# gvanhorn38/multibox

Measured on AMD Instinct MI355X. Metric: images/sec (299x299, 5-AR priors) train, higher is better.
Workload: dtype bf16; 1 GPU; full train step: Inception-ResNet-v2 + multibox heads fwd, on-device matching+loss, bwd, RMSProp+EMA; 299x299, k=5 (P=646), BATCH_SIZE=64/GPU, MAX_NUM_BBOXES=13; global_batch=64, parallelism=dp1, hip_graph=True

## Files before the change

multibox_amd/csrc/bn.hip:

```cpp
#include "vec8.h"
#include <string.h>
#include <type_traits>

namespace {

__device__ __forceinline__ void block_sum2(double& s1, double& s2) {
  __shared__ double red[kT / 64][2];
  s1 = wave_sum(s1); s2 = wave_sum(s2);
  if ((threadIdx.x & 63) == 0) { red[threadIdx.x >> 6][0] = s1; red[threadIdx.x >> 6][1] = s2; }
  __syncthreads();
  s1 = red[0][0] + red[1][0] + red[2][0] + red[3][0];
  s2 = red[0][1] + red[1][1] + red[2][1] + red[3][1];
}

__device__ __forceinline__ double bn_mean_var(double s1, double s2, double inv_count, double& var) {
  const double m = s1 * inv_count;
  var = s2 * inv_count - m * m;
  if (var < 0.0) var = 0.0;
  return m;
}
__device__ __forceinline__ float bn_rstd(double var, float eps) { return (float)(1.0 / sqrt(var + (double)eps)); }
__device__ __forceinline__ void bn_publish(int c, float fm, float fr, double var, float decay, float* mean,
                                           float* rstd, float* mmean, float* mvar) {
  mean[c] = fm;
// ... 445 lines not shown
      const float2 v1 = *reinterpret_cast<const float2*>(src + (size_t)(r + 1) * C * 2);
      const float2 v2 = *reinterpret_cast<const float2*>(src + (size_t)(r + 2) * C * 2);
      const float2 v3 = *reinterpret_cast<const float2*>(src + (size_t)(r + 3) * C * 2);
      s1 += ((double)v0.x + (double)v1.x) + ((double)v2.x + (double)v3.x);
      s2 += ((double)v0.y + (double)v1.y) + ((double)v2.y + (double)v3.y);
    }
    for (; r < rows; ++r) {
      const float2 v = *reinterpret_cast<const float2*>(src + (size_t)r * C * 2);
      s1 += v.x; s2 += v.y;
    }
    const float mu = mean[ch], rs = rstd[ch];
    const double sgx = (double)rs * (s2 - (double)mu * s1);
    s_par[ch] = mu; s_par[C + ch] = rs; s_par[2 * C + ch] = thr[ch];
    s_par[3 * C + ch] = (float)(s1 * inv_M); s_par[4 * C + ch] = (float)(sgx * inv_M);
    if (blockIdx.x == 0 && dbeta) dbeta[ch] += (float)s1;
  }
  __syncthreads();
  if (!active) return;
  float mu[8], rs[8], th[8], m1[8], m2[8];
#pragma unroll
  for (int j = 0; j < 8; ++j) {
    mu[j] = s_par[c + j]; rs[j] = s_par[C + c + j]; th[j] = s_par[2 * C + c + j]; m1[j] = s_par[3 * C + c + j]; m2[j] = s_par[4 * C + c + j];
  }
  u32x4 gc = g0, yc = y0;
  for (; m < M; m += step) {
    u32x4 gn = u32x4{0u, 0u, 0u, 0u}, yn = u32x4{0u, 0u, 0u, 0u};
    if (m + step < M) { gn = ld8(dap + (m + step) * ld_da); yn = ld8(y + (m + step) * C + c); }
    float g[8], yy[8], o[8];
    unpack8(gc, g);
    unpack8(yc, yy);
#pragma unroll
    for (int j = 0; j < 8; ++j)
      o[j] = bn_bwd_value(g[j], bn_xhat(yy[j], mu[j], rs[j]), yy[j] > th[j], rs[j], m1[j], m2[j]);
    st8(dy + m * C + c, pack8(o));
    gc = gn; yc = yn;
  }
}

inline unsigned rows_launch_grid(long long M, int C) {
  static const int rows_blocks = mbx_env_int("MBX_BN_ROWS_BLOCKS", 1024);
  const int C8 = C / 8, rpi = kT / C8 > 0 ? kT / C8 : 1;
  const long long g = (M + rpi - 1) / rpi;
  return (unsigned)(g > rows_blocks ? rows_blocks : g);
}

inline void bn_fused_grid(long long M, int C, int rows, int& groups, int& chunks, int& rpc) {
  groups = (C + kBnGroup - 1) / kBnGroup;
  static const int blocks_few = mbx_env_int("MBX_BN_FUSED_BLOCKS", 1024), blocks_many = mbx_env_int("MBX_BN_FUSED_BLOCKS_MANY", 256);
  long long want = (rows > 16 ? blocks_many : blocks_few) / groups;
  if (want < 1) want = 1;
  long long maxc = (M + 255) / 256;
  if (want > maxc) want = maxc;
  rpc = (int)((M + want - 1) / want);
  chunks = (int)((M + rpc - 1) / rpc);
}

#ifndef MBX_OB_SLOTS
#define MBX_OB_SLOTS 8
#endif
#ifndef MBX_OB_SLEEP
#define MBX_OB_SLEEP 8
#endif
constexpr int kObT = 512;
constexpr int kObSlots = MBX_OB_SLOTS;
constexpr int kObMaxNV = 20;
#ifndef MBX_OB_SUB
#define MBX_OB_SUB 16
#endif
#ifndef MBX_OB_REL
#define MBX_OB_REL 32
#endif
constexpr int kObSub = MBX_OB_SUB, kObRel = MBX_OB_REL, kObLine = 32;
constexpr int kObCtlWords = kObLine * (2 + kObSub + kObRel);

struct ObGeom { int C8, rpi, G, rpb, nv; };
inline ObGeom ob_geom(long long M, int C, int ncu) {
  ObGeom g;
  g.C8 = C / 8;
  g.rpi = g.C8 <= kObT ? kObT / g.C8 : 0;
  if (g.rpi == 0) { g.G = g.rpb = 0; g.nv = 1 << 30; return g; }
  long long G = (M + g.rpi - 1) / g.rpi;
  if (G > ncu) G = ncu;
  g.rpb = (int)((M + G - 1) / G);
  g.G = (int)((M + g.rpb - 1) / g.rpb);
  g.nv = (g.rpb + g.rpi - 1) / g.rpi;
  return g;
}

__device__ __forceinline__ unsigned ld_agent(const unsigned* p) {
  return __hip_atomic_load(p, __ATOMIC_RELAXED, __HIP_MEMORY_SCOPE_AGENT);
}
__device__ __forceinline__ float ld_agent(const float* p) {
  return __hip_atomic_load(p, __ATOMIC_RELAXED, __HIP_MEMORY_SCOPE_AGENT);
}

__device__ __forceinline__ __amdgpu_buffer_rsrc_t ob_rsrc(const void* p, unsigned bytes) {
  return __builtin_amdgcn_make_buffer_rsrc(const_cast<void*>(p), (short)0, (int)bytes, 0x00020000);
}
__device__ __forceinline__ u32x4 ob_load16(__amdgpu_buffer_rsrc_t r, unsigned byte_off) {
  return __builtin_amdgcn_raw_buffer_load_b128(r, (int)byte_off, 0, 0);
}
__device__ __forceinline__ void ob_store16(__amdgpu_buffer_rsrc_t r, unsigned byte_off, u32x4 v) {
  __builtin_amdgcn_raw_buffer_store_b128(v, r, (int)byte_off, 0, 0);
}

template <int NC, int NR>
__device__ __forceinline__ void ob_sum_cols(const float* p, int cstride, int ncols, int rstride, int nrows, float (&t)[NC]) {
#pragma unroll
  for (int k = 0; k < NC; ++k) t[k] = 0.f;
  for (int r0 = 0; r0 < nrows; r0 += NR) {
    float v[NC][NR];
#pragma unroll
    for (int k = 0; k < NC; ++k) {
      const int ko = (k < ncols ? k : 0) * cstride;
#pragma unroll
      for (int r = 0; r < NR; ++r) v[k][r] = p[ko + (r0 + r < nrows ? r0 + r : nrows - 1) * rstride];
    }
#pragma unroll
    for (int r = 0; r < NR; ++r) {
      const bool in = r0 + r < nrows;
#pragma unroll
      for (int k = 0; k < NC; ++k) t[k] += in ? v[k][r] : 0.f;
    }
  }
}

template <int NC, int NR>
__device__ __forceinline__ void ob_reduce_wide(const float* rows, int C2, int rpi, float* acc) {
  for (int e0 = threadIdx.x; e0 < C2; e0 += NC * kObT) {
    const int ncols = (C2 - e0 + kObT - 1) / kObT;
    float t[NC];
    ob_sum_cols<NC, NR>(rows + e0, kObT, ncols, C2, rpi, t);
#pragma unroll
    for (int k = 0; k < NC; ++k)
      if (k < ncols) atomicAdd(acc + e0 + k * kObT, t[k]);
  }
}

template <int NV, bool RELU>
__global__ void __launch_bounds__(kObT)
bn_bwd_onepass_kernel(const unsigned short* __restrict__ da, int ld_da, const unsigned short* __restrict__ y,
                      long long M, int C, const float* __restrict__ mean, const float* __restrict__ rstd,
                      const float* __restrict__ beta, float* __restrict__ dbeta, unsigned short* __restrict__ dy,
                      float* __restrict__ ws, int rpi, int rpb, float inv_M, unsigned spin_limit, int fault,
                      float* __restrict__ step_poison, const ChanMap map, int map_max) {
  extern __shared__ __attribute__((aligned(16))) float sred[];
  __shared__ int s_timeout;
  const int C8 = C >> 3;
  const int vc = threadIdx.x % C8, rr = threadIdx.x / C8;
  const bool active = rr < rpi;
  const int c = vc << 3;
  const long long r0 = (long long)((fault & 2) ? xcd_logical((int)blockIdx.x, (int)gridDim.x) : (int)blockIdx.x) * rpb;
  long long nr = (r0 + rpb > M ? M : r0 + rpb) - r0;
  const int nrows = nr > 0 ? (int)nr : 0;
  const __amdgpu_buffer_rsrc_t gr = ob_rsrc(da + r0 * ld_da, nrows ? (unsigned)(((nrows - 1) * ld_da + C + map_max) * 2) : 0u);
  const int cg = c + chan_off(map, c);
  const __amdgpu_buffer_rsrc_t yr = ob_rsrc(y + r0 * C, (unsigned)(nrows * C * 2));
  const __amdgpu_buffer_rsrc_t dr = ob_rsrc(dy + r0 * C, (unsigned)(nrows * C * 2));
  constexpr unsigned kPast = 0x80000000u;
  u32x4 vg[NV], vy[NV];
#pragma unroll
  for (int i = 0; i < NV; ++i) {
    const int lr = rr + i * rpi;
    const bool ok = active && lr < nrows;
    vg[i] = ob_load16(gr, ok ? (unsigned)((lr * ld_da + cg) * 2) : kPast);
    vy[i] = ob_load16(yr, ok ? (unsigned)((lr * C + c) * 2) : kPast);
  }
  float s1[8], s2[8], mu[8], rs[8], be[8];
  {
    const int cs = active ? c : 0;
    const float4 a0 = *reinterpret_cast<const float4*>(mean + cs), a1 = *reinterpret_cast<const float4*>(mean + cs + 4);
    const float4 b0 = *reinterpret_cast<const float4*>(rstd + cs), b1 = *reinterpret_cast<const float4*>(rstd + cs + 4);
    mu[0] = a0.x; mu[1] = a0.y; mu[2] = a0.z; mu[3] = a0.w; mu[4] = a1.x; mu[5] = a1.y; mu[6] = a1.z; mu[7] = a1.w;
    rs[0] = b0.x; rs[1] = b0.y; rs[2] = b0.z; rs[3] = b0.w; rs[4] = b1.x; rs[5] = b1.y; rs[6] = b1.z; rs[7] = b1.w;
    if (RELU) {
      const float4 c0 = *reinterpret_cast<const float4*>(beta + cs), c1 = *reinterpret_cast<const float4*>(beta + cs + 4);
      be[0] = c0.x; be[1] = c0.y; be[2] = c0.z; be[3] = c0.w; be[4] = c1.x; be[5] = c1.y; be[6] = c1.z; be[7] = c1.w;
    } else {
#pragma unroll
      for (int j = 0; j < 8; ++j) be[j] = 0.f;
    }
#pragma unroll
    for (int j = 0; j < 8; ++j) { s1[j] = 0.f; s2[j] = 0.f; }
  }
#pragma unroll
  for (int i = 0; i < NV; ++i) {
    asm volatile("" : "+v"(vg[i]), "+v"(vy[i]));
    float g[8], yy[8];
    unpack8(vg[i], g);
    unpack8(vy[i], yy);
#pragma unroll
    for (int j = 0; j < 8; ++j) {
      const float xh = bn_xhat(yy[j], mu[j], rs[j]);
      const float gj = (!RELU || bn_pre_relu(xh, be[j]) > 0.f) ? g[j] : 0.f;
      s1[j] += gj;
      s2[j] += gj * xh;
    }
    asm volatile("" : "+v"(s1[0]), "+v"(s1[1]), "+v"(s1[2]), "+v"(s1[3]), "+v"(s1[4]), "+v"(s1[5]), "+v"(s1[6]), "+v"(s1[7]));
    asm volatile("" : "+v"(s2[0]), "+v"(s2[1]), "+v"(s2[2]), "+v"(s2[3]), "+v"(s2[4]), "+v"(s2[5]), "+v"(s2[6]), "+v"(s2[7]));
  }
  const int C2 = 2 * C;
  if (active) {
    float4* o1 = reinterpret_cast<float4*>(sred + (size_t)rr * C2 + c);
    float4* o2 = reinterpret_cast<float4*>(sred + (size_t)rr * C2 + C + c);
    o1[0] = make_float4(s1[0], s1[1], s1[2], s1[3]); o1[1] = make_float4(s1[4], s1[5], s1[6], s1[7]);
    o2[0] = make_float4(s2[0], s2[1], s2[2], s2[3]); o2[1] = make_float4(s2[4], s2[5], s2[6], s2[7]);
  }
  __syncthreads();
  float* acc = ws + (size_t)(blockIdx.x & (kObSlots - 1)) * 2 * C;
  unsigned* ctl = reinterpret_cast<unsigned*>(ws + (size_t)kObSlots * 2 * C);
  const int np = C2 < kObT ? kObT / C2 : 1;
  if (np > 1) {
    float* part = sred + (size_t)rpi * C2;
    const int e = threadIdx.x % C2, p = threadIdx.x / C2;
    float t[1];
    if (p < np) {
      ob_sum_cols<1, 16>(sred + p * C2 + e, 0, 1, np * C2, (rpi - p + np - 1) / np, t);
      part[p * C2 + e] = t[0];
    }
    __syncthreads();
    if (threadIdx.x < C2) {
      ob_sum_cols<1, 16>(part + threadIdx.x, 0, 1, C2, np, t);
      atomicAdd(acc + threadIdx.x, t[0]);
    }
  } else if (rpi > 8) ob_reduce_wide<1, 16>(sred, C2, rpi, acc);
  else if (rpi > 4) ob_reduce_wide<2, 8>(sred, C2, rpi, acc);
  else if (rpi > 2) ob_reduce_wide<4, 4>(sred, C2, rpi, acc);
  else if (rpi > 1) ob_reduce_wide<8, 2>(sred, C2, rpi, acc);
  else ob_reduce_wide<16, 1>(sred, C2, rpi, acc);
  asm volatile("s_waitcnt vmcnt(0) lgkmcnt(0)" ::: "memory");
  __syncthreads();
  if (threadIdx.x == 0) {
    const unsigned G = gridDim.x, b = blockIdx.x;
    const unsigned sub = b % kObSub, n_sub = (G - sub + kObSub - 1) / kObSub, n_top = G < kObSub ? G : kObSub;
    s_timeout = 0;
    bool last = ((fault & 1) && b == 0) ? false : atomicAdd(ctl + kObLine * (1 + sub), 1u) == n_sub - 1;
    if (last) last = atomicAdd(ctl + kObLine * (1 + kObSub), 1u) == n_top - 1;
    if (last) {
      for (int r = 0; r < kObRel; ++r)
        __hip_atomic_store(ctl + kObLine * (2 + kObSub + r), 1u, __ATOMIC_RELAXED, __HIP_MEMORY_SCOPE_AGENT);
    } else {
      const unsigned* rel = ctl + kObLine * (2 + kObSub + b % kObRel);
      unsigned spins = 0;
      while (ld_agent(rel) == 0u) {
        __builtin_amdgcn_s_sleep(MBX_OB_SLEEP);
        if (++spins > spin_limit) {
          ctl[1] = 1u; s_timeout = 1;
          if (step_poison) atomicAdd(step_poison, 1.0f);
          break;
        }
      }
    }
    if (b == 0) ctl[0] = G;
  }
  __syncthreads();
  for (int e = threadIdx.x; e < 2 * C; e += kObT) {
    float t = 0.f;
#pragma unroll
    for (int sl = 0; sl < kObSlots; ++sl) t += ld_agent(ws + (size_t)sl * 2 * C + e);
    sred[e] = t;
  }
  __syncthreads();
  float m1[8], m2[8], t1[8];
  const float poison = s_timeout ? __builtin_nanf("") : 0.f;
  {
    const float* tot = sred + (active ? c : 0);
    u32x4 p0 = *reinterpret_cast<const u32x4*>(tot), p1 = *reinterpret_cast<const u32x4*>(tot + 4);
    u32x4 q0 = *reinterpret_cast<const u32x4*>(tot + C), q1 = *reinterpret_cast<const u32x4*>(tot + C + 4);
    asm volatile("" : "+v"(p0), "+v"(p1), "+v"(q0), "+v"(q1));
#pragma unroll
    for (int j = 0; j < 4; ++j) {
      t1[j] = __uint_as_float(p0[j]); t1[4 + j] = __uint_as_float(p1[j]);
      m2[j] = __uint_as_float(q0[j]); m2[4 + j] = __uint_as_float(q1[j]);
    }
  }
#pragma unroll
  for (int j = 0; j < 8; ++j) {
    t1[j] = (active ? t1[j] : 0.f) + poison;
    m1[j] = t1[j] * inv_M;
    m2[j] = (active ? m2[j] : 0.f) * inv_M;
  }
  if (blockIdx.x == 0 && rr == 0 && dbeta) {
#pragma unroll
    for (int j = 0; j < 8; ++j) atomicAdd(dbeta + c + j, t1[j]);
  }
#pragma unroll
  for (int i = 0; i < NV; ++i) {
    const int lr = rr + i * rpi;
    const bool ok = active && lr < nrows;
    asm volatile("" : "+v"(vg[i]), "+v"(vy[i]));
    float g[8], yy[8], o[8];
    unpack8(vg[i], g);
    unpack8(vy[i], yy);
#pragma unroll
    for (int j = 0; j < 8; ++j) {
      const float xh = bn_xhat(yy[j], mu[j], rs[j]);
      o[j] = bn_bwd_value(g[j], xh, !RELU || bn_pre_relu(xh, be[j]) > 0.f, rs[j], m1[j], m2[j]);
    }
    ob_store16(dr, ok ? (unsigned)((lr * C + c) * 2) : kPast, pack8(o));
    asm volatile("" ::: "memory");
  }
}

__global__ void __launch_bounds__(kT)
bn_apply_maxpool3s2_kernel(const unsigned short* __restrict__ y, int N, int H, int W, int C, const float* __restrict__ mean,
                           const float* __restrict__ rstd, const float* __restrict__ beta, int relu,
                           unsigned short* __restrict__ p, long long ps, int ldp, int Ho, int Wo,
                           unsigned char* __restrict__ argmax) {
  const int C8 = C >> 3;
  const unsigned total = (unsigned)N * Ho * Wo * C8;
  for (unsigned i = blockIdx.x * kT + threadIdx.x; i < total; i += gridDim.x * kT) {
    unsigned t = i / (unsigned)C8;
    const int c = (int)(i - t * C8) << 3;
    const unsigned t2 = t / (unsigned)Wo;
    const int ow = (int)(t - t2 * Wo);
    const int n = (int)(t2 / (unsigned)Ho);
    const int oh = (int)(t2 - (unsigned)n * Ho);
    u32x4 v[9];
#pragma unroll
    for (int r = 0; r < 3; ++r)
#pragma unroll
      for (int q = 0; q < 3; ++q)
        v[r * 3 + q] = ld8(y + (((long long)n * H + (oh * 2 + r)) * W + (ow * 2 + q)) * C + c);
    float mu[8], rs[8], be[8], best[8];
    unsigned arg[8];
#pragma unroll
    for (int j = 0; j < 8; ++j) { mu[j] = mean[c + j]; rs[j] = rstd[c + j]; be[j] = beta[c + j]; best[j] = -INFINITY; arg[j] = 0; }
#pragma unroll
    for (int tq = 0; tq < 9; ++tq) {
      float f[8];
      unpack8(v[tq], f);
#pragma unroll
      for (int j = 0; j < 8; ++j) {
        const float a = bf2f(f2bf(bn_fwd_value(f[j], mu[j], rs[j], be[j], relu)));
        if (a > best[j]) { best[j] = a; arg[j] = tq; }
      }
    }
    st8(p + n * ps + ((long long)oh * Wo + ow) * ldp + c, pack8(best));
    if (argmax) {
      u32x2 av;
      av.x = arg[0] | (arg[1] << 8) | (arg[2] << 16) | (arg[3] << 24);
      av.y = arg[4] | (arg[5] << 8) | (arg[6] << 16) | (arg[7] << 24);
      *reinterpret_cast<u32x2*>(argmax + (((long long)n * Ho + oh) * Wo + ow) * C + c) = av;
    }
  }
}

struct PoolSrc { const unsigned short* gy; long long gys; int ld_gy; const unsigned char* argmax; int H, W, Ho, Wo, C, Hb, Wb; };
__device__ __forceinline__ void pool3s2_grad_block(const PoolSrc& p, int n, int a, int b, int c, float (&g)[4][8]) {
  u32x4 gv[4];
  u32x2 av[4];
  bool ok[4];
#pragma unroll
  for (int i = 0; i < 4; ++i) {
    const int oh = a - 1 + (i >> 1), ow = b - 1 + (i & 1);
    const bool v = oh >= 0 && oh < p.Ho && ow >= 0 && ow < p.Wo;
    ok[i] = v;
    const long long o = ((long long)n * p.Ho + (v ? oh : 0)) * p.Wo + (v ? ow : 0);
    av[i] = v ? *reinterpret_cast<const u32x2*>(p.argmax + o * p.C + c) : u32x2{0xffffffffu, 0xffffffffu};
    gv[i] = v ? ld8(p.gy + n * p.gys + ((long long)oh * p.Wo + ow) * p.ld_gy + c) : u32x4{0u, 0u, 0u, 0u};
  }
  float w[4][8];
#pragma unroll
  for (int i = 0; i < 4; ++i) unpack8(gv[i], w[i]);
  (void)ok;
#pragma unroll
  for (int j = 0; j < 8; ++j) {
    unsigned t[4];
#pragma unroll
    for (int i = 0; i < 4; ++i) t[i] = ((j < 4 ? av[i].x : av[i].y) >> (8 * (j & 3))) & 0xffu;
    float p00 = 0.f, p01 = 0.f, p10 = 0.f, p11 = 0.f;
    if (t[0] == 8u) p00 += w[0][j];
    if (t[1] == 6u) p00 += w[1][j];
    if (t[2] == 2u) p00 += w[2][j];
    if (t[3] == 0u) p00 += w[3][j];
    if (t[1] == 7u) p01 += w[1][j];
    if (t[3] == 1u) p01 += w[3][j];
    if (t[2] == 5u) p10 += w[2][j];
    if (t[3] == 3u) p10 += w[3][j];
    if (t[3] == 4u) p11 += w[3][j];
    g[0][j] = bf2f(f2bf(p00)); g[1][j] = bf2f(f2bf(p01)); g[2][j] = bf2f(f2bf(p10)); g[3][j] = bf2f(f2bf(p11));
  }
}

template <bool RELU>
__global__ void __launch_bounds__(kT)
bn_bwd_reduce_pool_kernel(const PoolSrc ps, const unsigned short* __restrict__ y, long long Mb, int C,
                          const float* __restrict__ mean, const float* __restrict__ rstd, const float* __restrict__ beta,
                          int rpi, int rpb, float* __restrict__ partial) {
  extern __shared__ __attribute__((aligned(16))) float sred[];
  const int C8 = C >> 3;
  const int vc = threadIdx.x % C8, rr = threadIdx.x / C8;
  const bool active = rr < rpi;
  const int c = vc << 3;
  float s1[8], s2[8], mu[8], rs[8], be[8];
#pragma unroll
  for (int j = 0; j < 8; ++j) {
    s1[j] = 0.f; s2[j] = 0.f; mu[j] = mean[c + j]; rs[j] = rstd[c + j];
    be[j] = RELU ? beta[c + j] : 0.f;
  }
  const long long r0 = (long long)blockIdx.x * rpb;
  long long r1 = r0 + rpb;
  if (r1 > Mb) r1 = Mb;
  const unsigned HWb = (unsigned)(ps.Hb * ps.Wb);
  if (active)
    for (long long m = r0 + rr; m < r1; m += rpi) {
      const unsigned mu_ = (unsigned)m, n = mu_ / HWb, rem = mu_ - n * HWb, a = rem / (unsigned)ps.Wb, b = rem - a * (unsigned)ps.Wb;
      u32x4 yv[4];
      bool in[4];
#pragma unroll
      for (int q = 0; q < 4; ++q) {
        const int h = 2 * (int)a + (q >> 1), w = 2 * (int)b + (q & 1);
        in[q] = h < ps.H && w < ps.W;
        yv[q] = ld8(y + (((long long)n * ps.H + (h < ps.H ? h : ps.H - 1)) * ps.W + (w < ps.W ? w : ps.W - 1)) * C + c);
      }
      float g[4][8];
      pool3s2_grad_block(ps, (int)n, (int)a, (int)b, c, g);
#pragma unroll
      for (int q = 0; q < 4; ++q) {
        float yy[8];
        unpack8(yv[q], yy);
#pragma unroll
        for (int j = 0; j < 8; ++j) {
          const float xh = bn_xhat(yy[j], mu[j], rs[j]);
          const float gj = (in[q] && bn_relu_pass<RELU ? 2 : 0>(0.f, xh, be[j])) ? g[q][j] : 0.f;
          s1[j] += gj;
          s2[j] += gj * xh;
        }
      }
    }
  bn_bwd_reduce_epilogue(sred, C8, rpi, vc, rr, active, s1, s2, C, partial);
}

template <bool RELU>
__global__ void __launch_bounds__(kT)
bn_bwd_apply_pool_kernel(const PoolSrc ps, const unsigned short* __restrict__ y, long long Mb, int C, long long M,
                         const float* __restrict__ mean, const float* __restrict__ rstd, const float* __restrict__ beta,
                         const float* __restrict__ m12, unsigned short* __restrict__ dy) {
  const int C8 = C >> 3;
  const long long total = Mb * C8;
  const unsigned HWb = (unsigned)(ps.Hb * ps.Wb);
  for (long long i = (long long)blockIdx.x * kT + threadIdx.x; i < total; i += (long long)gridDim.x * kT) {
    const long long m = i / C8;
    const int c = (int)(i - m * C8) << 3;
    const unsigned mu_ = (unsigned)m, n = mu_ / HWb, rem = mu_ - n * HWb, a = rem / (unsigned)ps.Wb, b = rem - a * (unsigned)ps.Wb;
    float g[4][8], mu[8], rs[8], be[8], q1[8], q2[8];
#pragma unroll
    for (int j = 0; j < 8; ++j) {
      mu[j] = mean[c + j]; rs[j] = rstd[c + j]; be[j] = RELU ? beta[c + j] : 0.f; q1[j] = m12[c + j]; q2[j] = m12[C + c + j];
    }
    u32x4 yv[4];
#pragma unroll
    for (int q = 0; q < 4; ++q) {
      const int h = 2 * (int)a + (q >> 1), w = 2 * (int)b + (q & 1);
      yv[q] = ld8(y + (((long long)n * ps.H + (h < ps.H ? h : ps.H - 1)) * ps.W + (w < ps.W ? w : ps.W - 1)) * C + c);
    }
    pool3s2_grad_block(ps, (int)n, (int)a, (int)b, c, g);
#pragma unroll
    for (int q = 0; q < 4; ++q) {
      const int h = 2 * (int)a + (q >> 1), w = 2 * (int)b + (q & 1);
      if (h >= ps.H || w >= ps.W) continue;
      const long long row = ((long long)n * ps.H + h) * ps.W + w;
      float yy[8], o[8];
      unpack8(yv[q], yy);
#pragma unroll
      for (int j = 0; j < 8; ++j) {
        const float xh = bn_xhat(yy[j], mu[j], rs[j]);
        o[j] = bn_bwd_value(g[q][j], xh, bn_relu_pass<RELU ? 2 : 0>(0.f, xh, be[j]), rs[j], q1[j], q2[j]);
      }
      st8(dy + row * C + c, pack8(o));
    }
  }
}

__global__ void __launch_bounds__(kT)
bn_moving_update_kernel(float* __restrict__ mm, float* __restrict__ mv, const float* __restrict__ bmean,
                        const float* __restrict__ bvar, long long n, float decay, const float* __restrict__ skip_ctl,
                        unsigned long long* __restrict__ skipped, float* __restrict__ ema_m, float* __restrict__ ema_v,
                        float ema_d) {
  if (skip_ctl && (skip_ctl[0] != 0.f || skip_ctl[1] != 0.f)) {
    if (skipped && blockIdx.x == 0 && threadIdx.x == 0) *skipped += 1ull;
    return;
  }
  for (long long i = (long long)blockIdx.x * kT + threadIdx.x; i < n; i += (long long)gridDim.x * kT) {
    const float m = mm[i] - (1.0f - decay) * (mm[i] - bmean[i]);
    const float v = mv[i] - (1.0f - decay) * (mv[i] - bvar[i]);
    mm[i] = m;
    mv[i] = v;
    if (ema_m) { const float e = ema_m[i]; ema_m[i] = e - (1.0f - ema_d) * (e - m); }
    if (ema_v) { const float e = ema_v[i]; ema_v[i] = e - (1.0f - ema_d) * (e - v); }
  }
}

}

extern "C" int mbx_bn_finalize(const float* part, int rows, int C, int64_t count, float eps, float decay, float* mean,
                               float* rstd, float* mmean, float* mvar, mbx_stream_t stream) {
  if (!part || !mean || !rstd || rows <= 0 || C <= 0 || count <= 0) return MBX_ERR_INVALID_ARG;
  MBX_ENTER();
  hipLaunchKernelGGL(bn_finalize_kernel, dim3(C), dim3(kT), 0, mbx_s(stream), part, rows, C,
                     1.0 / (double)count, eps, decay, mean, rstd, mmean, mvar);
  MBX_LAUNCH_CHECK();
  return MBX_OK;
}

extern "C" int mbx_bn_fold(const float* mm, const float* mv, const float* beta, float eps, int C, float* scale,
                           float* shift, mbx_stream_t stream) {
  if (!mm || !mv || !scale || !shift || C <= 0) return MBX_ERR_INVALID_ARG;
  MBX_ENTER();
  hipLaunchKernelGGL(bn_fold_kernel, dim3((C + kT - 1) / kT), dim3(kT), 0, mbx_s(stream), mm, mv, beta, eps, C, scale, shift);
  MBX_LAUNCH_CHECK();
  return MBX_OK;
}

static int to_chan_map(const mbx_chan_map* m, int C, ChanMap& out) {
  memset(&out, 0, sizeof(out));
  if (!m) return MBX_OK;
  if (m->n < 0 || m->n > 4) return MBX_ERR_INVALID_ARG;
  for (int i = 0; i < m->n; ++i) {
    if (m->c_begin[i] % 8 || m->offset[i] % 8 || m->offset[i] < 0 || m->c_begin[i] >= C ||
        (i == 0 ? m->c_begin[0] != 0 : m->c_begin[i] <= m->c_begin[i - 1]))
      return MBX_ERR_INVALID_ARG;
    out.cb[i] = m->c_begin[i]; out.off[i] = m->offset[i];
  }
  out.n = m->n;
  return MBX_OK;
}

extern "C" int mbx_bn_apply_mapped(const void* y, int64_t M, int C, const float* mean, const float* rstd, const float* beta,
                                   int relu, void* a, int ld_a, const mbx_chan_map* map, mbx_stream_t stream) {
  if (!y || !a || !mean || !rstd || !beta || M <= 0 || C <= 0 || C % 8 || ld_a % 8 || !al16(y) || !al16(a))
    return MBX_ERR_INVALID_ARG;
  ChanMap cm;
  if (to_chan_map(map, C, cm) != MBX_OK) return MBX_ERR_INVALID_ARG;
  MBX_ENTER();
  hipLaunchKernelGGL(bn_apply_kernel, dim3(grid_for(M * (C / 8))), dim3(kT), 0, mbx_s(stream), (cus)y, (long long)M, C,
                     mean, rstd, beta, relu, (us)a, ld_a, cm);
  MBX_LAUNCH_CHECK();
  return MBX_OK;
}

extern "C" int mbx_bn_apply(const void* y, int64_t M, int C, const float* mean, const float* rstd, const float* beta,
                            int relu, void* a, int ld_a, mbx_stream_t stream) {
  return mbx_bn_apply_mapped(y, M, C, mean, rstd, beta, relu, a, ld_a, nullptr, stream);
}

extern "C" int mbx_bn_finalize_parts(const float* const* parts, const int32_t* rows, const int32_t* Cs, int n_parts,
                                     int64_t count, float eps, float decay, float* mean, float* rstd, float* mmean,
                                     float* mvar, mbx_stream_t stream) {
  if (!parts || !rows || !Cs || n_parts <= 0 || n_parts > 4 || !mean || !rstd || count <= 0) return MBX_ERR_INVALID_ARG;
  PartTable t;
  memset(&t, 0, sizeof(t));
  int c = 0;
  for (int i = 0; i < n_parts; ++i) {
    if (!parts[i] || rows[i] <= 0 || Cs[i] <= 0) return MBX_ERR_INVALID_ARG;
    t.part[i] = parts[i]; t.rows[i] = rows[i]; t.C[i] = Cs[i]; t.cstart[i] = c;
    c += Cs[i];
  }
  for (int i = n_parts; i <= 4; ++i) t.cstart[i] = c;
  t.n = n_parts;
  MBX_ENTER();
  hipLaunchKernelGGL(bn_finalize_parts_kernel, dim3(c), dim3(kT), 0, mbx_s(stream), t, 1.0 / (double)count, eps, decay, mean,
                     rstd, mmean, mvar);
  MBX_LAUNCH_CHECK();
  return MBX_OK;
}

extern "C" int mbx_bn_bwd_rows(int64_t M, int C) {
  if (M <= 0 || C <= 0 || C % 8 || C > 2048) return MBX_ERR_INVALID_ARG;
  return bn_bwd_geom(M, C).rows;
}

static int bn_bwd_args_ok(const void* da, int ld_da, const void* a, int ld_a, int relu, const void* y, int64_t M, int C,
                          const float* mean, const float* rstd, const float* beta) {
  if (!da || !y || !mean || !rstd || (relu && !a && !beta) || M <= 0 || C <= 0 || C % 8 || ld_da % 8 || (a && ld_a % 8))
    return 0;
  return al16(da) && al16(y) && (!a || al16(a));
}

extern "C" int mbx_bn_bwd_reduce(const void* da, int ld_da, const void* a, int ld_a, int relu, const void* y, int64_t M,
                                 int C, const float* mean, const float* rstd, const float* beta, float* partial,
                                 mbx_stream_t stream) {
  return mbx_bn_bwd_reduce_mapped(da, ld_da, a, ld_a, relu, y, M, C, mean, rstd, beta, partial, nullptr, stream);
}

extern "C" int mbx_bn_bwd_reduce_mapped(const void* da, int ld_da, const void* a, int ld_a, int relu, const void* y, int64_t M,
                                        int C, const float* mean, const float* rstd, const float* beta, float* partial,
                                        const mbx_chan_map* da_map, mbx_stream_t stream) {
  if (!partial || !bn_bwd_args_ok(da, ld_da, a, ld_a, relu, y, M, C, mean, rstd, beta)) return MBX_ERR_INVALID_ARG;
  if (C > 2048) return MBX_ERR_UNSUPPORTED;
  ChanMap cm;
  if (to_chan_map(da_map, C, cm) != MBX_OK || (da_map && da_map->n && a)) return MBX_ERR_INVALID_ARG;
  const BnBwdGeom g = bn_bwd_geom(M, C);
  MBX_ENTER();
  with_relu_mask(relu, a, [&](auto mask) {
    hipLaunchKernelGGL(bn_bwd_reduce_kernel<decltype(mask)::value>, dim3(g.rows), dim3(kT), reduce_lds_bytes(g), mbx_s(stream),
                       (cus)da, ld_da, (cus)a, ld_a, (cus)y, (long long)M, C, mean, rstd, beta, g.rows_per_iter, g.rpb, partial, cm);
  });
  MBX_LAUNCH_CHECK();
  return MBX_OK;
}

extern "C" int mbx_bn_bwd_finalize(const float* partial, int rows, int C, int64_t M, float* dbeta, float* m12,
                                   mbx_stream_t stream) {
  if (!partial || !m12 || rows <= 0 || C <= 0 || M <= 0) return MBX_ERR_INVALID_ARG;
  MBX_ENTER();
  hipLaunchKernelGGL(bn_bwd_finalize_kernel, dim3(C), dim3(kT), 0, mbx_s(stream), partial, rows, C,
                     1.0 / (double)M, dbeta, m12);
  MBX_LAUNCH_CHECK();
  return MBX_OK;
}

extern "C" int mbx_bn_bwd_apply(const void* da, int ld_da, const void* a, int ld_a, int relu, const void* y, int64_t M,
                                int C, const float* mean, const float* rstd, const float* beta, const float* m12,
                                void* dy, mbx_stream_t stream) {
  return mbx_bn_bwd_apply_mapped(da, ld_da, a, ld_a, relu, y, M, C, mean, rstd, beta, m12, dy, nullptr, stream);
}

extern "C" int mbx_bn_bwd_apply_mapped(const void* da, int ld_da, const void* a, int ld_a, int relu, const void* y, int64_t M,
                                       int C, const float* mean, const float* rstd, const float* beta, const float* m12,
                                       void* dy, const mbx_chan_map* da_map, mbx_stream_t stream) {
  if (!m12 || !dy || !al16(dy) || !bn_bwd_args_ok(da, ld_da, a, ld_a, relu, y, M, C, mean, rstd, beta))
    return MBX_ERR_INVALID_ARG;
  ChanMap cm;
  if (to_chan_map(da_map, C, cm) != MBX_OK || (da_map && da_map->n && a)) return MBX_ERR_INVALID_ARG;
  MBX_ENTER();
  with_relu_mask(relu, a, [&](auto mask) {
    hipLaunchKernelGGL(bn_bwd_apply_kernel<decltype(mask)::value>, dim3(grid_for(M * (C / 8))), dim3(kT), 0, mbx_s(stream), (cus)da,
                       ld_da, (cus)a, ld_a, (cus)y, (long long)M, C, mean, rstd, beta, m12, (us)dy, cm);
  });
  MBX_LAUNCH_CHECK();
  return MBX_OK;
}

extern "C" int mbx_bn_bwd_apply_rows(const float* stats, int rows, const void* da, int ld_da, const void* y, int64_t M, int C,
                                     const float* mean, const float* rstd, const float* relu_thr, float* dbeta, void* dy,
                                     const mbx_chan_map* da_map, mbx_stream_t stream) {
  if (!stats || rows <= 0 || rows > 16 || !da || !y || !mean || !rstd || !relu_thr || !dy || M <= 0 || C <= 0 || C % 8 ||
      ld_da % 8 || !al16(da) || !al16(y) || !al16(dy) || !al16(stats))
    return MBX_ERR_INVALID_ARG;
  if (C > kRowsMaxC) return MBX_ERR_UNSUPPORTED;
  ChanMap cm;
  if (to_chan_map(da_map, C, cm) != MBX_OK) return MBX_ERR_INVALID_ARG;
  MBX_ENTER();
  hipLaunchKernelGGL(bn_bwd_rows_kernel, dim3(rows_launch_grid(M, C)), dim3(kT), (size_t)5 * C * sizeof(float), mbx_s(stream), stats, rows,
                     1.0 / (double)M, (cus)da, ld_da, (cus)y, (long long)M, C, mean, rstd, relu_thr, dbeta, (us)dy, cm);
  MBX_LAUNCH_CHECK();
  return MBX_OK;
}

extern "C" size_t mbx_bn_bwd_onepass_workspace_bytes(int C) {
  return C > 0 ? ((size_t)kObSlots * 2 * C + kObCtlWords) * sizeof(float) : 0;
}

static int ob_groups(int max_workgroups) {
  const int ncu = mbx_cu_count();
  return (max_workgroups > 0 && max_workgroups < ncu) ? max_workgroups : ncu;
}

extern "C" int mbx_bn_bwd_onepass_supported(int64_t M, int C, int max_workgroups) {
  if (M <= 0 || C <= 0 || C % 8) return 0;
  const int ncu = ob_groups(max_workgroups);
  if (ncu <= 0) return 0;
  return ob_geom(M, C, ncu).nv <= kObMaxNV;
}

extern "C" int mbx_bn_bwd_onepass(const void* da, int ld_da, int relu, const void* y, int64_t M, int C, const float* mean,
                                  const float* rstd, const float* beta, float* dbeta, void* dy, void* ws,
                                  int max_workgroups, float* step_poison, mbx_stream_t stream) {
  return mbx_bn_bwd_onepass_mapped(da, ld_da, relu, y, M, C, mean, rstd, beta, dbeta, dy, ws, max_workgroups, step_poison,
                                   nullptr, stream);
}

extern "C" int mbx_bn_bwd_onepass_mapped(const void* da, int ld_da, int relu, const void* y, int64_t M, int C,
                                         const float* mean, const float* rstd, const float* beta, float* dbeta, void* dy,
                                         void* ws, int max_workgroups, float* step_poison, const mbx_chan_map* da_map,
                                         mbx_stream_t stream) {
  ChanMap cm;
  if (C <= 0 || to_chan_map(da_map, C, cm) != MBX_OK) return MBX_ERR_INVALID_ARG;
  const int map_max = chan_map_max(cm);
  if (!da || !y || !mean || !rstd || (relu && !beta) || !dy || !ws || M <= 0 || C <= 0 || C % 8 || ld_da % 8 || !al16(da) ||
      !al16(y) || !al16(dy) || !al16(ws) || !al16(mean) || !al16(rstd) || (relu && !al16(beta)))
    return MBX_ERR_INVALID_ARG;
  const int ncu = ob_groups(max_workgroups);
  if (ncu <= 0) return MBX_ERR_LAUNCH;
  const ObGeom g = ob_geom(M, C, ncu);
  if (g.nv > kObMaxNV) return MBX_ERR_UNSUPPORTED;
  MBX_ENTER();
  const size_t lds = ((size_t)g.rpi * 2 * C + (size_t)(2 * C > kObT ? 2 * C : kObT)) * sizeof(float);
  const int fault = mbx_barrier_fault() == '1';
  const unsigned spin_limit = fault ? (1u << 10) : (1u << 22);
#define MBX_OB(NV, RELU)                                                                                               \
  hipLaunchKernelGGL((bn_bwd_onepass_kernel<NV, RELU>), dim3(g.G), dim3(kObT), lds, mbx_s(stream), (cus)da, ld_da,      \
                     (cus)y, (long long)M, C, mean, rstd, beta, dbeta, (us)dy, (float*)ws, g.rpi, g.rpb,               \
                     (float)(1.0 / (double)M), spin_limit, fault | (xcd_rows_on() << 1), step_poison, cm, map_max)
#define MBX_OB_NV(NV) do { if (relu) MBX_OB(NV, true); else MBX_OB(NV, false); } while (0)
  if (g.nv <= 2) MBX_OB_NV(2);
  else if (g.nv <= 4) MBX_OB_NV(4);
  else if (g.nv <= 8) MBX_OB_NV(8);
  else if (g.nv <= 12) MBX_OB_NV(12);
  else if (g.nv <= 16) MBX_OB_NV(16);
  else MBX_OB_NV(20);
#undef MBX_OB_NV
#undef MBX_OB
  MBX_LAUNCH_CHECK();
  return MBX_OK;
}

static bool pool3s2_shape_ok(int H, int W, int Ho, int Wo) { return Ho == (H - 3) / 2 + 1 && Wo == (W - 3) / 2 + 1; }

static int pool_src_ok(const void* gy, int ld_gy, const uint8_t* argmax, int N, int H, int W, int Ho, int Wo, int C, PoolSrc& ps,
                       int64_t gys) {
  if (!gy || !argmax || N <= 0 || H <= 0 || W <= 0 || C <= 0 || C % 8 || ld_gy % 8 || !al16(gy) || (reinterpret_cast<uintptr_t>(argmax) & 7))
    return MBX_ERR_INVALID_ARG;
  if (!pool3s2_shape_ok(H, W, Ho, Wo)) return MBX_ERR_INVALID_ARG;
  if ((long long)N * H * W >= (1LL << 31)) return MBX_ERR_UNSUPPORTED;
  ps.gy = (cus)gy; ps.gys = gys; ps.ld_gy = ld_gy; ps.argmax = argmax; ps.H = H; ps.W = W; ps.Ho = Ho; ps.Wo = Wo; ps.C = C;
  ps.Hb = (H + 1) / 2; ps.Wb = (W + 1) / 2;
  return MBX_OK;
}

extern "C" int mbx_bn_apply_maxpool(const void* y, int N, int H, int W, int C, const float* mean, const float* rstd,
                                    const float* beta, int relu, void* p, int64_t p_img_stride, int ld_p, int Ho, int Wo,
                                    uint8_t* argmax, mbx_stream_t stream) {
  if (!y || !p || !mean || !rstd || !beta || N <= 0 || H < 3 || W < 3 || C <= 0 || C % 8 || ld_p % 8 || !al16(y) || !al16(p) ||
      (argmax && (reinterpret_cast<uintptr_t>(argmax) & 7)))
    return MBX_ERR_INVALID_ARG;
  if (!pool3s2_shape_ok(H, W, Ho, Wo)) return MBX_ERR_INVALID_ARG;
  if ((long long)N * Ho * Wo * (C / 8) >= (1LL << 31) || (long long)N * H * W * C >= (1LL << 40)) return MBX_ERR_UNSUPPORTED;
  MBX_ENTER();
  hipLaunchKernelGGL(bn_apply_maxpool3s2_kernel, dim3(grid_for((long long)N * Ho * Wo * (C / 8))), dim3(kT), 0, mbx_s(stream),
                     (cus)y, N, H, W, C, mean, rstd, beta, relu, (us)p, (long long)p_img_stride, ld_p, Ho, Wo, argmax);
  MBX_LAUNCH_CHECK();
  return MBX_OK;
}

extern "C" int mbx_bn_bwd_rows_pooled(int N, int H, int W, int C) {
  if (N <= 0 || H <= 0 || W <= 0 || C <= 0 || C % 8 || C > 2048) return MBX_ERR_INVALID_ARG;
  return bn_bwd_geom((long long)N * ((H + 1) / 2) * ((W + 1) / 2), C).rows;
}

extern "C" int mbx_bn_bwd_reduce_pooled(const void* gy, int64_t gy_img_stride, int ld_gy, const uint8_t* argmax, int N, int H,
                                        int W, int Ho, int Wo, int relu, const void* y, int C, const float* mean,
                                        const float* rstd, const float* beta, float* partial, mbx_stream_t stream) {
  PoolSrc ps;
  int st = pool_src_ok(gy, ld_gy, argmax, N, H, W, Ho, Wo, C, ps, gy_img_stride);
  if (st != MBX_OK) return st;
  if (!y || !al16(y) || !mean || !rstd || (relu && !beta) || !partial || C > 2048) return MBX_ERR_INVALID_ARG;
  const long long Mb = (long long)N * ps.Hb * ps.Wb;
  const BnBwdGeom g = bn_bwd_geom(Mb, C);
  MBX_ENTER();
  with_relu(relu, [&](auto on) {
    hipLaunchKernelGGL(bn_bwd_reduce_pool_kernel<decltype(on)::value>, dim3(g.rows), dim3(kT), reduce_lds_bytes(g), mbx_s(stream), ps,
                       (cus)y, Mb, C, mean, rstd, beta, g.rows_per_iter, g.rpb, partial);
  });
  MBX_LAUNCH_CHECK();
  return MBX_OK;
}

extern "C" int mbx_bn_bwd_apply_pooled(const void* gy, int64_t gy_img_stride, int ld_gy, const uint8_t* argmax, int N, int H,
                                       int W, int Ho, int Wo, int relu, const void* y, int C, const float* mean,
                                       const float* rstd, const float* beta, const float* m12, void* dy, mbx_stream_t stream) {
  PoolSrc ps;
  int st = pool_src_ok(gy, ld_gy, argmax, N, H, W, Ho, Wo, C, ps, gy_img_stride);
  if (st != MBX_OK) return st;
  if (!y || !al16(y) || !mean || !rstd || (relu && !beta) || !m12 || !dy || !al16(dy)) return MBX_ERR_INVALID_ARG;
  const long long M = (long long)N * H * W, Mb = (long long)N * ps.Hb * ps.Wb;
  MBX_ENTER();
  with_relu(relu, [&](auto on) {
    hipLaunchKernelGGL(bn_bwd_apply_pool_kernel<decltype(on)::value>, dim3(grid_for(Mb * (C / 8))), dim3(kT), 0, mbx_s(stream), ps,
                       (cus)y, Mb, C, M, mean, rstd, beta, m12, (us)dy);
  });
  MBX_LAUNCH_CHECK();
  return MBX_OK;
}

extern "C" int mbx_bn_moving_update(float* moving_mean, float* moving_var, const float* batch_mean, const float* batch_var,
                                    int64_t n, float decay, const float* skip_ctl, uint64_t* skipped_steps,
                                    float* ema_mean, float* ema_var, float ema_decay, mbx_stream_t stream) {
  if (!moving_mean || !moving_var || !batch_mean || !batch_var || n <= 0 || decay < 0.f) return MBX_ERR_INVALID_ARG;
  MBX_ENTER();
  hipLaunchKernelGGL(bn_moving_update_kernel, dim3(grid_for(n)), dim3(kT), 0, mbx_s(stream), moving_mean, moving_var,
                     batch_mean, batch_var, (long long)n, decay, skip_ctl, reinterpret_cast<unsigned long long*>(skipped_steps),
                     ema_mean, ema_var, ema_decay);
  MBX_LAUNCH_CHECK();
  return MBX_OK;
}

extern "C" int mbx_bn_apply_fused_mapped(const void* stats_partial, int rows, int64_t count, float eps, float decay,
                                         const void* y, int64_t M, int C, const float* beta, int relu, void* a, int ld_a,
                                         const mbx_chan_map* a_map, float* mean, float* rstd, float* mmean, float* mvar,
                                         float* relu_thr, mbx_stream_t stream) {
  if (!stats_partial || !y || !a || !beta || !mean || !rstd || rows <= 0 || M <= 0 || C <= 0 || C % 8 || ld_a % 8 ||
      count <= 0 || !al16(y) || !al16(a) || !al16(stats_partial))
    return MBX_ERR_INVALID_ARG;
  if (rows > 16 || C > kRowsMaxC) return MBX_ERR_UNSUPPORTED;
  ChanMap cm;
  if (to_chan_map(a_map, C, cm) != MBX_OK) return MBX_ERR_INVALID_ARG;
  MBX_ENTER();
  hipLaunchKernelGGL(bn_apply_rows_kernel, dim3(rows_launch_grid(M, C)), dim3(kT), (size_t)3 * C * sizeof(float), mbx_s(stream),
                     reinterpret_cast<const float*>(stats_partial), rows, 1.0 / (double)count, eps, decay, (cus)y, (long long)M, C,
                     beta, relu, (us)a, ld_a, mean, rstd, mmean, mvar, cm, relu_thr, xcd_rows_on());
  MBX_LAUNCH_CHECK();
  return MBX_OK;
}

extern "C" int mbx_bn_apply_fused(const float* stats_partial, int rows, int64_t count, float eps, float decay, const void* y,
                                  int64_t M, int C, const float* beta, int relu, void* a, int ld_a, float* mean,
                                  float* rstd, float* mmean, float* mvar, mbx_stream_t stream) {
  if (!stats_partial || !y || !a || !beta || !mean || !rstd || rows <= 0 || M <= 0 || C <= 0 || C % 8 || ld_a % 8 ||
      count <= 0 || !al16(y) || !al16(a))
    return MBX_ERR_INVALID_ARG;
  static const int fused_rows = mbx_env_int("MBX_BN_FUSED_ROWS", 16);
  static const long long fused_elems = mbx_env_int("MBX_BN_FUSED_KELEMS", 6200) * 1000LL;
  if (rows > 16 && (rows > fused_rows || M * C > fused_elems)) {
    int st = mbx_bn_finalize(stats_partial, rows, C, count, eps, decay, mean, rstd, mmean, mvar, stream);
    if (st != MBX_OK) return st;
    return mbx_bn_apply(y, M, C, mean, rstd, beta, relu, a, ld_a, stream);
  }
  MBX_ENTER();
  int groups, chunks, rpc;
  bn_fused_grid(M, C, rows, groups, chunks, rpc);
  hipLaunchKernelGGL(bn_apply_fused_kernel, dim3(groups, chunks), dim3(kT), 0, mbx_s(stream), stats_partial, rows,
                     1.0 / (double)count, eps, decay, (cus)y, (long long)M, C, beta, relu, (us)a, ld_a, mean, rstd, mmean,
                     mvar, rpc, ChanMap{}, nullptr);
  MBX_LAUNCH_CHECK();
  return MBX_OK;
}
```

Before: 4415 images/sec.

## Compute 2x2 pooled outputs per thread in fused BN+maxpool with row prefetch

The fused BN-apply + 3x3 stride-2 maxpool kernel now has each thread produce a 2x2 block of output pixels from a 5x5 input window. Overlapping input pixels are loaded and normalized once instead of up to four times, and the per-channel BN parameters are hoisted out of the pixel loop. The next input row is prefetched into registers while the current one is processed, and the relu flag becomes a template parameter. In exchange the kernel uses more registers and clamps edge columns and rows in more complex index logic.

```diff
diff --git a/multibox_amd/csrc/bn.hip b/multibox_amd/csrc/bn.hip
--- a/multibox_amd/csrc/bn.hip
+++ b/multibox_amd/csrc/bn.hip
@@ -771,46 +771,86 @@
   }
 }
 
+template <bool RELU>
 __global__ void __launch_bounds__(kT)
 bn_apply_maxpool3s2_kernel(const unsigned short* __restrict__ y, int N, int H, int W, int C, const float* __restrict__ mean,
-                           const float* __restrict__ rstd, const float* __restrict__ beta, int relu,
+                           const float* __restrict__ rstd, const float* __restrict__ beta,
                            unsigned short* __restrict__ p, long long ps, int ldp, int Ho, int Wo,
                            unsigned char* __restrict__ argmax) {
   const int C8 = C >> 3;
-  const unsigned total = (unsigned)N * Ho * Wo * C8;
-  for (unsigned i = blockIdx.x * kT + threadIdx.x; i < total; i += gridDim.x * kT) {
-    unsigned t = i / (unsigned)C8;
-    const int c = (int)(i - t * C8) << 3;
-    const unsigned t2 = t / (unsigned)Wo;
-    const int ow = (int)(t - t2 * Wo);
-    const int n = (int)(t2 / (unsigned)Ho);
-    const int oh = (int)(t2 - (unsigned)n * Ho);
-    u32x4 v[9];
-#pragma unroll
-    for (int r = 0; r < 3; ++r)
-#pragma unroll
-      for (int q = 0; q < 3; ++q)
-        v[r * 3 + q] = ld8(y + (((long long)n * H + (oh * 2 + r)) * W + (ow * 2 + q)) * C + c);
-    float mu[8], rs[8], be[8], best[8];
-    unsigned arg[8];
-#pragma unroll
-    for (int j = 0; j < 8; ++j) { mu[j] = mean[c + j]; rs[j] = rstd[c + j]; be[j] = beta[c + j]; best[j] = -INFINITY; arg[j] = 0; }
-#pragma unroll
-    for (int tq = 0; tq < 9; ++tq) {
-      float f[8];
-      unpack8(v[tq], f);
-#pragma unroll
-      for (int j = 0; j < 8; ++j) {
-        const float a = bf2f(f2bf(bn_fwd_value(f[j], mu[j], rs[j], be[j], relu)));
-        if (a > best[j]) { best[j] = a; arg[j] = tq; }
+  const int rpi = C8 <= kT ? kT / C8 : 1;
+  const int rr = threadIdx.x / C8;
+  if (rr >= rpi) return;
+  const int cstep = C8 <= kT ? C8 : kT;
+  const unsigned Hb = (unsigned)(Ho + 1) >> 1, Wb = (unsigned)(Wo + 1) >> 1;
+  const unsigned nblk = (unsigned)N * Hb * Wb;
+  for (int vc = threadIdx.x - rr * C8; vc < C8; vc += cstep) {
+    const int c = vc << 3;
+    float mu[8], rs[8], be[8];
+#pragma unroll
+    for (int j = 0; j < 8; ++j) { mu[j] = mean[c + j]; rs[j] = rstd[c + j]; be[j] = beta[c + j]; }
+    for (unsigned m = blockIdx.x * rpi + rr; m < nblk; m += gridDim.x * rpi) {
+      const unsigned t = m / Wb, bw = m - t * Wb, n = t / Hb, bh = t - n * Hb;
+      const int oh = 2 * (int)bh, ow = 2 * (int)bw;
+      const bool row1 = oh + 1 < Ho, col1 = ow + 1 < Wo;
+      const unsigned short* yc[5];
+#pragma unroll
+      for (int q = 0; q < 5; ++q) {
+        const int w = 2 * ow + q;
+        yc[q] = y + (((long long)n * H + 2 * oh) * W + (w < W ? w : W - 1)) * C + c;
       }
-    }
-    st8(p + n * ps + ((long long)oh * Wo + ow) * ldp + c, pack8(best));
-    if (argmax) {
-      u32x2 av;
-      av.x = arg[0] | (arg[1] << 8) | (arg[2] << 16) | (arg[3] << 24);
-      av.y = arg[4] | (arg[5] << 8) | (arg[6] << 16) | (arg[7] << 24);
-      *reinterpret_cast<u32x2*>(argmax + (((long long)n * Ho + oh) * Wo + ow) * C + c) = av;
+      const long long rstride = (long long)W * C, rstride34 = row1 ? rstride : 0;
+      float best[4][8];
+      unsigned arg[4][8];
+#pragma unroll
+      for (int o = 0; o < 4; ++o)
+#pragma unroll
+        for (int j = 0; j < 8; ++j) { best[o][j] = -INFINITY; arg[o][j] = 0; }
+      u32x4 cur[5], nxt[5];
+#pragma unroll
+      for (int q = 0; q < 5; ++q) cur[q] = ld8(yc[q]);
+#pragma unroll
+      for (int r = 0; r < 5; ++r) {
+        if (r + 1 < 5) {
+#pragma unroll
+          for (int q = 0; q < 5; ++q) nxt[q] = ld8(yc[q] + (r + 1 < 3 ? (r + 1) * rstride : 2 * rstride + (r - 1) * rstride34));
+        }
+        asm volatile("" ::: "memory");
+        {
+#pragma unroll
+          for (int q = 0; q < 5; ++q) {
+            float f[8], a[8];
+            unpack8(cur[q], f);
+#pragma unroll
+            for (int j = 0; j < 8; ++j) f[j] = bn_fwd_value(f[j], mu[j], rs[j], be[j], RELU);
+            unpack8(pack8(f), a);
+#pragma unroll
+            for (int o = 0; o < 4; ++o) {
+              const int wr = r - 2 * (o >> 1), wq = q - 2 * (o & 1);
+              if (wr < 0 || wr > 2 || wq < 0 || wq > 2) continue;
+#pragma unroll
+              for (int j = 0; j < 8; ++j) {
+                if (a[j] > best[o][j]) { best[o][j] = a[j]; arg[o][j] = (unsigned)(wr * 3 + wq); }
+                asm volatile("" : "+v"(best[o][j]), "+v"(arg[o][j]));
+              }
+            }
+          }
+        }
+#pragma unroll
+        for (int q = 0; q < 5; ++q) cur[q] = nxt[q];
+      }
+#pragma unroll
+      for (int o = 0; o < 4; ++o) {
+        if (((o >> 1) && !row1) || ((o & 1) && !col1)) continue;
+        const long long pix = (long long)(oh + (o >> 1)) * Wo + (ow + (o & 1));
+        st8(p + n * ps + pix * ldp + c, pack8(best[o]));
+        if (argmax) {
+          u32x2 av;
+          av.x = arg[o][0] | (arg[o][1] << 8) | (arg[o][2] << 16) | (arg[o][3] << 24);
+          av.y = arg[o][4] | (arg[o][5] << 8) | (arg[o][6] << 16) | (arg[o][7] << 24);
+          *reinterpret_cast<u32x2*>(argmax + ((long long)n * Ho * Wo + pix) * C + c) = av;
+        }
+      }
     }
   }
 }
@@ -1197,9 +1237,13 @@
     return MBX_ERR_INVALID_ARG;
   if (!pool3s2_shape_ok(H, W, Ho, Wo)) return MBX_ERR_INVALID_ARG;
   if ((long long)N * Ho * Wo * (C / 8) >= (1LL << 31) || (long long)N * H * W * C >= (1LL << 40)) return MBX_ERR_UNSUPPORTED;
-  MBX_ENTER();
-  hipLaunchKernelGGL(bn_apply_maxpool3s2_kernel, dim3(grid_for((long long)N * Ho * Wo * (C / 8))), dim3(kT), 0, mbx_s(stream),
-                     (cus)y, N, H, W, C, mean, rstd, beta, relu, (us)p, (long long)p_img_stride, ld_p, Ho, Wo, argmax);
+  const int C8 = C / 8, rpi = C8 <= kT ? kT / C8 : 1;
+  const long long nblk = (long long)N * ((Ho + 1) / 2) * ((Wo + 1) / 2);
+  MBX_ENTER();
+  with_relu(relu, [&](auto on) {
+    hipLaunchKernelGGL(bn_apply_maxpool3s2_kernel<decltype(on)::value>, dim3(grid_for((nblk + rpi - 1) / rpi * kT)), dim3(kT), 0,
+                       mbx_s(stream), (cus)y, N, H, W, C, mean, rstd, beta, (us)p, (long long)p_img_stride, ld_p, Ho, Wo, argmax);
+  });
   MBX_LAUNCH_CHECK();
   return MBX_OK;
 }
```

Measured after the change: 4424 images/sec, median of 3. About the same (+0.2%).
